# flo-audio/flo

Measured on AMD Instinct MI355X. Metric: Msamples/s encoded (44.1k stereo, q=high), higher is better.
Workload: dtype f32

## Files before the change

### diag/lds_model.py

```python
#!/usr/bin/env python3
import argparse
import re
from collections import Counter

import numpy as np

N, HOP, NB = 2048, 1024, 25
SLOT_CAP = 96
ROW = 1024
EDGES = np.array([0, 100, 200, 300, 400, 510, 630, 770, 920, 1080, 1270, 1480, 1720, 2000, 2320, 2700, 3150, 3700,
                  4400, 5300, 6400, 7700, 9500, 12000, 15500, 20500], dtype=np.float32)

R_WIN, R_TW, R_F1, R_F2, R_LANE, R_KEEP, R_DST, R_S10 = 0, 8, 12, 16, 20, 21, 25, 32


def bands(rate):
    res = np.float32(rate) / np.float32(N)
    band = []
    for k in range(HOP):
        f = (np.float32(k) + np.float32(0.5)) * res
        b = NB - 1
        for i in range(1, 26):
            if f < EDGES[i]:
                b = i - 1
                break
        band.append(b)
    return band


def band_tables(rate):
    band = bands(rate)
    lane_bnd, lane_slot0, slot_band = [0] * 64, [0] * 64, []
    for j in range(64):
        lane_slot0[j] = len(slot_band)
        for e in range(16):
            k = 16 * j + e
            if e == 15 or band[k + 1] != band[k]:
                lane_bnd[j] |= 1 << e
                slot_band.append(band[k])
    dirty = 0
    for m in lane_bnd:
        dirty |= m
    band_slot0, s = [], 0
    for b in range(NB):
        band_slot0.append(s)
        while s < len(slot_band) and slot_band[s] == b:
            s += 1
    band_slot0.append(s)
    return lane_bnd, lane_slot0, band_slot0, dirty


G128 = [[0, 1, 2, 3, 12, 13, 14, 15] + list(range(20, 28)), [4, 5, 6, 7, 8, 9, 10, 11, 16, 17, 18, 19] + list(range(28, 32))]
G128 = G128 + [[l + 32 for l in g] for g in G128]
G32 = [list(range(0, 32)), list(range(32, 64))]


def contig(n):
    return [list(range(i, i + n)) for i in range(0, 64, n)]


RULES = {
    "ds_read_b32": [(G32, 1, 32)], "ds_write_b32": [(G32, 1, 32)], "ds_write_b16": [(G32, 1, 32)],
    "ds_read_b64": [(G32, 2, 64)], "ds_read_b128": [(G128, 4, 64)],
    "ds_read2_b32": [(G32, 1, 32), (G32, 1, 32)], "ds_write2_b32": [(G32, 1, 32), (G32, 1, 32)],
    "ds_read2_b64": [(contig(16), 2, 32), (contig(16), 2, 32)],
    "ds_write_b64": [(contig(16), 2, 32)], "ds_write_b128": [(contig(8), 4, 32)],
    "ds_write2_b64": [(contig(16), 2, 32), (contig(16), 2, 32)],
}
SKIP_EMPTY = False
GATHER_MASKS = False


def cost(kind, addrs):
    acc = RULES[kind]
    lists = addrs if len(acc) == 2 else [addrs]
    cyc = base = 0
    for (groups, dw, nbank), ad in zip(acc, lists):
        for g in groups:
            per_bank = {}
            for l in g:
                if ad[l] is None:
                    continue
                for i in range(dw):
                    d = ad[l] // 4 + i
                    per_bank.setdefault(d % nbank, set()).add(d)
            if SKIP_EMPTY and not per_bank:
                continue
            cyc += max([len(v) for v in per_bank.values()] or [1])
            base += 1
    return cyc, cyc - base


def lanes(f):
    return [f(l) for l in range(64)]


def sites(rate, layout):
    lane_bnd, lane_slot0, band_slot0, dirty = band_tables(rate)
    row = lambda r, off=0: lanes(lambda l: r * ROW + 16 * l + off)
    uni = lambda a: lanes(lambda l: a)
    one = lambda a: [a] + [None] * 63
    S = []
    S += [("frame", "peek consumed / coef counters", "ds_read_b32", uni(0x8000))] * 2
    S += [("frame", "kRowS10 (uniform)", "ds_read_b128", uni(R_S10 * ROW))] * 2
    if layout == "old":
        S += [("frame", "rcount: kRowLane .z", "ds_read_b32", row(R_LANE, 8))]
    else:
        S += [("frame", "rcount: kRowS10 dword 64 + lane", "ds_read_b32", lanes(lambda l: R_S10 * ROW + 256 + 4 * l))]
    for ph, rr in (("fft pass 1", R_F1), ("fft pass 2", R_F2)):
        S += [(ph, "twiddle rows", "ds_read_b128", row(rr + k)) for k in range(3)]
        S += [(ph, "twiddle row 4 (.xy)", "ds_read_b64", row(rr + 3))]
    X = 0x10000
    for ka in range(8):
        S += [("fft exchange 1", "writes", "ds_write_b128", lanes(lambda l: X + 16 * ((8 * ka + (l & 7)) * 9 + (l >> 3))))]
    for r in range(8):
        S += [("fft exchange 1", "reads", "ds_read_b128", lanes(lambda l: X + 16 * (l * 9 + r)))]
    T = X + 16000
    S += [("masking pass", "ts_ready peek", "ds_read_b32", uni(0x8004))]
    S += [("masking pass", "ts (tl, sf)", "ds_write2_b32", [lanes(lambda l: T + 16 * (l & 31) + 4 * (l >> 5) + o if (l & 31) < 25 else None) for o in (0, 8)])]
    S += [("masking pass", "sfwh", "ds_write_b16", lanes(lambda l: T + 1024 + 2 * l if (l & 31) < 25 else None))]
    S += [("masking pass", "alive", "ds_write_b64", one(T + 1200))]
    S += [("masking pass", "ts_ready", "ds_write_b32", one(0x8004))]
    for kb in range(8):
        S += [("fft exchange 2", "writes", "ds_write_b128", lanes(lambda l: X + 16 * (((l >> 3) + 8 * kb) * 9 + (l & 7))))]
    for r in range(8):
        S += [("fft exchange 2", "reads", "ds_read_b128", lanes(lambda l: X + 16 * (l * 9 + r)))]
    pl = lambda l: 2 * l + 2 * (l >> 3)
    for r in range(8):
        if layout == "old" or r % 2 == 0:
            if layout == "old":
                S += [("post-rotation", "twiddle rows (half rows)", "ds_read_b64", row(R_TW + r // 2, 8 * (r & 1)))]
            elif layout != "carry":
                S += [("post-rotation", "twiddle rows", "ds_read_b128", row(R_TW + r // 2))]
        S += [("post-rotation", "transpose writes (2m)", "ds_write_b64", lanes(lambda l: X + 8 * (pl(l) + 144 * r)))]
        S += [("post-rotation", "transpose writes (1023-2m)", "ds_write_b64", lanes(lambda l: X + 8 * (1149 - pl(l) - 144 * r)))]
    for q in range(8):
        S += [("post-rotation", "transpose reads", "ds_read_b128", lanes(lambda l: X + 16 * (9 * l) + 16 * q))]
    S += [("band statistics", "coef_ready", "ds_write_b32", one(0x8008))]
    es = [e for e in range(16) if (dirty >> e) & 1]
    if layout == "old":
        for rr in (R_KEEP, R_DST):
            for g in range(4):
                comp = [e - 4 * g for e in es if 4 * g <= e < 4 * g + 4 and (rr == R_DST or e < 15)]
                i = 0
                while i < len(comp):
                    if i + 1 < len(comp) and comp[i + 1] == comp[i] + 1 and comp[i] % 2 == 1:
                        S += [("band statistics", "keep / dst rows (dword pieces)", "ds_read2_b32", [row(rr + g, 4 * comp[i]), row(rr + g, 4 * comp[i] + 4)])]
                        i += 2
                    elif i + 1 < len(comp) and comp[i + 1] == comp[i] + 1:
                        S += [("band statistics", "keep / dst rows (dword pieces)", "ds_read_b64", row(rr + g, 4 * comp[i]))]
                        i += 2
                    else:
                        S += [("band statistics", "keep / dst rows (dword pieces)", "ds_read_b32", row(rr + g, 4 * comp[i]))]
                        i += 1
    elif layout == "new":
        S += [("band statistics", "keep / dst rows (whole rows)", "ds_read_b128", row(rr + g)) for rr in (R_KEEP, R_DST) for g in range(4)]
    SL = X + 9216
    masks = layout in ("masks", "carry")
    for e in es:
        def dst(l, e=e, off=0):
            m = lane_bnd[l]
            if (m >> e) & 1:
                return SL + 16 * (lane_slot0[l] + bin(m & ((1 << e) - 1)).count("1")) + off
            return None if masks else SL + 16 * (SLOT_CAP + l)
        if masks and e == 15:
            S += [("band statistics", "slot store (element 15, all lanes)", "ds_write_b128", lanes(dst))]
        elif masks:
            S += [("band statistics", "slot stores (closing lanes)", "ds_write2_b64", [lanes(dst), lanes(lambda l: dst(l, off=8))])]
        else:
            S += [("band statistics", "slot stores", "ds_write_b128", lanes(dst))]
    zero = SLOT_CAP + 64
    for u in range(12):
        def src(l, u=u):
            b = min(l & 31, 24)
            bs0 = band_slot0[b] + (l >> 5)
            bs1 = band_slot0[b + 1] if (l & 31) < 25 else 0
            s = bs0 + 2 * u
            if masks and GATHER_MASKS and not bs0 + 2 * 4 * (u // 4) < bs1:
                return None
            return SL + 16 * (s if s < bs1 else zero)
        S += [("band statistics", "slot gathers", "ds_read_b128", lanes(src))]
    for r in range(8):
        S += [("fold", "window rows", "ds_read_b128", row(R_WIN + r))]
    if layout == "old":
        for k in range(4):
            S += [("fold", "twiddle rows (read2_b64)", "ds_read2_b64", [row(R_TW + k), row(R_TW + k, 8)])]
    elif layout != "carry":
        S += [("fold", "twiddle rows", "ds_read_b128", row(R_TW + k)) for k in range(4)]
    return S


def isa_mix(path):
    txt = open(path).read().split("\n")
    start = next(i for i, t in enumerate(txt) if re.match(r"^_ZN3flo20lossy_chain2q_kernelILb0ELj(\d+)ELb0EE.*:", t)
                 and "Lj65535E" not in t)
    body = txt[start:]
    e = next(i for i, t in enumerate(body) if re.match(r"^\.LBB\d+_\d+:.*_clEjS\d_S\d_S\d_S\d_\.exit", t))
    a = max(i for i, t in enumerate(body[:e]) if re.match(r"^\.LBB\d+_\d+:\s+; %\.lr\.ph\d*$", t))
    lab = body[e].split(":")[0]
    c = next(i for i, t in enumerate(body) if i > a and re.search(r"s_cbranch\w*\s+" + re.escape(lab) + r"\b", t))
    b = next(i for i, t in enumerate(body) if i > e and re.match(r"^\.LBB", t))
    mix, cold = Counter(), Counter()
    for i in range(a, b):
        m = re.search(r"\b(ds_[a-z0-9_]+)", body[i])
        if m:
            (cold if c <= i < e else mix)[m.group(1)] += 1
    return mix, cold


def main():
    ap = argparse.ArgumentParser()
    ap.add_argument("--rate", type=int, default=44100)
    ap.add_argument("--layout", default="old", choices=["old", "new", "masks", "carry"])
    ap.add_argument("--skip-empty", action="store_true")
    ap.add_argument("--gather-masks", action="store_true")
    ap.add_argument("--isa")
    a = ap.parse_args()
    global SKIP_EMPTY, GATHER_MASKS
    SKIP_EMPTY, GATHER_MASKS = a.skip_empty, a.gather_masks
    S = sites(a.rate, a.layout)
    tab = {}
    tot_c = tot_x = 0
    for ph, site, kind, ad in S:
        c, x = cost(kind, ad)
        k = (ph, site, kind)
        n, cc, xx = tab.get(k, (0, 0, 0))
        tab[k] = (n + 1, cc + c, xx + x)
        tot_c += c
        tot_x += x
    print(f"{'phase':16} {'site':38} {'instruction':14} {'n':>3} {'array':>6} {'conflict':>8}")
    for (ph, site, kind), (n, c, x) in tab.items():
        print(f"{ph:16} {site:38} {kind:14} {n:3d} {c:6d} {x:8d}")
    print(f"{'transform wave, one stereo frame':70} {len(S):3d} {tot_c:6d} {tot_x:8d}")
    if a.isa:
        mix, cold = isa_mix(a.isa)
        model = Counter(kind for _, _, kind, _ in S)
        print("ISA mix (one frame):", dict(sorted(mix.items())), " cold loop (not run at this rate):", dict(cold))
        print("model mix          :", dict(sorted(model.items())))


if __name__ == "__main__":
    main()
```

### flo_amd/csrc/lossy_device.hpp

```cpp
#pragma once
#include <hip/hip_runtime.h>
#include <stdint.h>

#include "pack_rows.h"

namespace flo {


struct LossyDevTables {
    const float4 *pack;
    const float4 *pack_g;
    const float4 *pack_ext;
    const float *ath_db;
    const uint8_t *band;
    const float *band_count;
    const float *s10d;
    const uint32_t *lane_bnd;
    const uint32_t *lane_slot0;
    const uint32_t *band_slot0;
    int max_band_slots;
    uint32_t dirty;
    float smr_thr;
    int q_transparent;
};
// ... 325 lines not shown
template <int CH>
__device__ __forceinline__ void post_rotate_transpose(const int lane, const float (&zr)[CH][8], const float (&zi)[CH][8],
                                                      float (*coef)[kCoefFloats], float (&c)[CH][16],
                                                      const LossyDevTables &T) {
#pragma unroll
    for (int r = 0; r < 8; r++) {
        const int m = lane + 64 * r;
        const float4 t4 = T.pack[(kRowTw + (r >> 1)) * 64 + lane];
        const float2 w = (r & 1) ? make_float2(t4.z, t4.w) : make_float2(t4.x, t4.y);
        const int k0 = 2 * m, k1 = 1023 - 2 * m;
        const int p0 = k0 + 4 * (k0 >> 5), p1 = k1 + 4 * (k1 >> 5);
#pragma unroll
        for (int ch = 0; ch < CH; ch++) {
            float R = fmaf(-zi[ch][r], w.y, -(zr[ch][r] * w.x));
            float I = fmaf(zi[ch][r], w.x, -(zr[ch][r] * w.y));
            coef[ch][p0] = R;
            coef[ch][p1] = I;
        }
    }
    wave_sync();
#pragma unroll
    for (int ch = 0; ch < CH; ch++) {
        const float4 *p = reinterpret_cast<const float4 *>(&coef[ch][16 * lane + 4 * (lane >> 1)]);
#pragma unroll
        for (int q = 0; q < 4; q++) {
            float4 v = p[q];
            c[ch][4 * q + 0] = v.x;
            c[ch][4 * q + 1] = v.y;
            c[ch][4 * q + 2] = v.z;
            c[ch][4 * q + 3] = v.w;
        }
    }
    wave_sync();
}

typedef float v2f __attribute__((ext_vector_type(2)));
typedef float v4f __attribute__((ext_vector_type(4)));
__device__ __forceinline__ v4f pack_row_v(const float4 *p) {
    v4f v = *reinterpret_cast<const v4f *>(p);
    asm("" : "+v"(v));
    return v;
}
__device__ __forceinline__ v2f fma2(v2f a, v2f b, v2f c) { return __builtin_elementwise_fma(a, b, c); }
__device__ __forceinline__ v2f fma2_na_hi_nc(v2f a, v2f w, v2f c) {
    v2f r;
    asm("v_pk_fma_f32 %0, %1, %2, %3 op_sel:[0,1,0] op_sel_hi:[1,1,1] neg_lo:[1,0,1] neg_hi:[1,0,1]" : "=v"(r) : "v"(a), "v"(w), "v"(c));
    return r;
}
__device__ __forceinline__ v2f fma2_a_hi_c(v2f a, v2f w, v2f c) {
    v2f r;
    asm("v_pk_fma_f32 %0, %1, %2, %3 op_sel:[0,1,0] op_sel_hi:[1,1,1]" : "=v"(r) : "v"(a), "v"(w), "v"(c));
    return r;
}
__device__ __forceinline__ v2f mul2_hi(v2f a, v2f w) {
    v2f r;
    asm("v_pk_mul_f32 %0, %1, %2 op_sel:[0,1] op_sel_hi:[1,1]" : "=v"(r) : "v"(a), "v"(w));
    return r;
}
__device__ __forceinline__ v2f fma2_a_hi_nc(v2f a, v2f w, v2f c) {
    v2f r;
    asm("v_pk_fma_f32 %0, %1, %2, %3 op_sel:[0,1,0] op_sel_hi:[1,1,1] neg_lo:[0,0,1] neg_hi:[0,0,1]" : "=v"(r) : "v"(a), "v"(w), "v"(c));
    return r;
}
__device__ __forceinline__ v2f mul2_lo(v2f a, v2f w) {
    v2f r;
    asm("v_pk_mul_f32 %0, %1, %2 op_sel:[0,0] op_sel_hi:[1,0]" : "=v"(r) : "v"(a), "v"(w));
    return r;
}
__device__ __forceinline__ v2f fma2_a_lo_nc(v2f a, v2f w, v2f c) {
    v2f r;
    asm("v_pk_fma_f32 %0, %1, %2, %3 op_sel:[0,0,0] op_sel_hi:[1,0,1] neg_lo:[0,0,1] neg_hi:[0,0,1]" : "=v"(r) : "v"(a), "v"(w), "v"(c));
    return r;
}
__device__ __forceinline__ v2f splat2(float x) { return (v2f){x, x}; }

constexpr int kXch4 = 64 * kXchStride;
constexpr int kCoef2 = 1024 + 2 * 64;

__device__ __forceinline__ void dft8_2(v2f *xr, v2f *xi) {
    const v2f s = splat2(0.70710678118654752440f);
    v2f a0r = xr[0] + xr[4], a0i = xi[0] + xi[4];
    v2f a1r = xr[0] - xr[4], a1i = xi[0] - xi[4];
    v2f a2r = xr[2] + xr[6], a2i = xi[2] + xi[6];
    v2f a3r = xr[2] - xr[6], a3i = xi[2] - xi[6];
    v2f a4r = xr[1] + xr[5], a4i = xi[1] + xi[5];
    v2f a5r = xr[1] - xr[5], a5i = xi[1] - xi[5];
    v2f a6r = xr[3] + xr[7], a6i = xi[3] + xi[7];
    v2f a7r = xr[3] - xr[7], a7i = xi[3] - xi[7];
    v2f b0r = a0r + a2r, b0i = a0i + a2i;
    v2f b2r = a0r - a2r, b2i = a0i - a2i;
    v2f b1r = a1r + a3i, b1i = a1i - a3r;
    v2f b3r = a1r - a3i, b3i = a1i + a3r;
    v2f c0r = a4r + a6r, c0i = a4i + a6i;
    v2f c2r = a4r - a6r, c2i = a4i - a6i;
    v2f c1r = a5r + a7i, c1i = a5i - a7r;
    v2f c3r = a5r - a7i, c3i = a5i + a7r;
    const v2f e1r = c1r + c1i, e1i = c1i - c1r;
    const v2f e3r = c3i - c3r, e3i = c3r + c3i;
    xr[0] = b0r + c0r; xi[0] = b0i + c0i;
    xr[4] = b0r - c0r; xi[4] = b0i - c0i;
    xr[1] = fma2(e1r, s, b1r); xi[1] = fma2(e1i, s, b1i);
    xr[5] = fma2(-e1r, s, b1r); xi[5] = fma2(-e1i, s, b1i);
    xr[2] = b2r + c2i; xi[2] = b2i - c2r;
    xr[6] = b2r - c2i; xi[6] = b2i + c2r;
    xr[3] = fma2(e3r, s, b3r); xi[3] = fma2(-e3i, s, b3i);
    xr[7] = fma2(-e3r, s, b3r); xi[7] = fma2(e3i, s, b3i);
}

__device__ __forceinline__ void cmul_2(v2f &xr, v2f &xi, float wr, float wi) {
    const v2f WR = splat2(wr), WI = splat2(wi);
    v2f r = fma2(xr, WR, -(xi * WI));
    v2f i = fma2(xr, WI, xi * WR);
    xr = r;
    xi = i;
}
__device__ __forceinline__ void cmul_2_pair(v2f &xr, v2f &xi, v2f w) {
    const v2f WR = splat2(w.x);
    v2f r = fma2(xr, WR, -mul2_hi(xi, w));
    v2f i = fma2_a_hi_c(xr, w, xi * WR);
    xr = r;
    xi = i;
}

struct NoShadow { __device__ __forceinline__ void operator()() const {} };
template <typename F = NoShadow>
__device__ __forceinline__ void fft512_2(const int lane, v2f (&zr)[8], v2f (&zi)[8], float4 *x4, const LossyDevTables &T, F &&shadow = F()) {
    dft8_2(zr, zi);
#pragma unroll
    for (int kk = 0; kk < 4; kk++) {
        const float4 w = T.pack[(kRowF1 + kk) * 64 + lane];
        cmul_2(zr[2 * kk + 1], zi[2 * kk + 1], w.x, w.y);
        if (kk < 3) cmul_2_pair(zr[2 * kk + 2], zi[2 * kk + 2], (v2f){w.z, w.w});
    }
    {
        const int nb = lane >> 3, nc = lane & 7;
#pragma unroll
        for (int ka = 0; ka < 8; ka++) x4[(8 * ka + nc) * kXchStride + nb] = make_float4(zr[ka].x, zr[ka].y, zi[ka].x, zi[ka].y);
        wave_sync();
#pragma unroll
        for (int r = 0; r < 8; r++) {
            const float4 v = x4[lane * kXchStride + r];
            zr[r] = (v2f){v.x, v.y};
            zi[r] = (v2f){v.z, v.w};
        }
        shadow();
        wave_sync();
    }
    dft8_2(zr, zi);
#pragma unroll
    for (int kk = 0; kk < 4; kk++) {
        const float4 w = T.pack[(kRowF2 + kk) * 64 + lane];
        cmul_2(zr[2 * kk + 1], zi[2 * kk + 1], w.x, w.y);
        if (kk < 3) cmul_2_pair(zr[2 * kk + 2], zi[2 * kk + 2], (v2f){w.z, w.w});
    }
    {
        const int ka = lane >> 3, nc = lane & 7;
#pragma unroll
        for (int kb = 0; kb < 8; kb++) x4[(ka + 8 * kb) * kXchStride + nc] = make_float4(zr[kb].x, zr[kb].y, zi[kb].x, zi[kb].y);
        wave_sync();
#pragma unroll
        for (int r = 0; r < 8; r++) {
            const float4 v = x4[lane * kXchStride + r];
            zr[r] = (v2f){v.x, v.y};
            zi[r] = (v2f){v.z, v.w};
        }
        wave_sync();
    }
    dft8_2(zr, zi);
}

__device__ __forceinline__ void load_half_fast_2(const int lane, const float *__restrict__ pcm, long long s0, v2f (&he)[8], v2f (&ho)[8]) {
    const char *base0 = reinterpret_cast<const char *>(pcm + s0 * 2);
    const char *base1 = base0 + 4096;
    const unsigned va = 16u * (unsigned)lane, vb = 16u * (unsigned)(63 - lane);
#pragma unroll
    for (int r = 0; r < 8; r++) {
        const int rr = r & 3;
        const char *pe = (r < 4 ? base1 : base0) + va + 1024 * rr;
        const char *po = (r < 4 ? base0 : base1) + vb + (3080 - 1024 * rr);
        const float2 a = *reinterpret_cast<const float2 *>(pe);
        const float2 b = *reinterpret_cast<const float2 *>(po);
        he[r] = (v2f){a.x, a.y};
        ho[r] = (v2f){b.x, b.y};
    }
}

__device__ __forceinline__ void fold_2(const int lane, const v2f (&ae)[8], const v2f (&ao)[8], const v2f (&be)[8], const v2f (&bo)[8],
                                       v2f (&zr)[8], v2f (&zi)[8], const LossyDevTables &T) {
    float4 t4;
#pragma unroll
    for (int r = 0; r < 8; r++) {
        const float4 ww = T.pack[(kRowWin + r) * 64 + lane];
        const v2f wae = splat2(ww.x), wao = splat2(ww.y), wbe = splat2(ww.z);
        const v2f whi = {ww.z, ww.w};
        if (!(r & 1)) t4 = pack_row(&T.pack[(kRowTw + (r >> 1)) * 64 + lane]);
        const v2f wx = splat2((r & 1) ? t4.z : t4.x);
        const v2f thi = {t4.z, t4.w};
        v2f re, im;
        if (r < 4) {
            re = fma2_na_hi_nc(bo[r], whi, be[r] * wbe);
            im = fma2(ao[r], wao, -(ae[r] * wae));
        } else {
            re = fma2(-ao[r], wao, ae[r] * wae);
            im = fma2_na_hi_nc(bo[r], whi, be[r] * wbe);
        }
        if (r & 1) {
            zr[r] = fma2_na_hi_nc(im, thi, re * wx);
            zi[r] = fma2_a_hi_nc(re, thi, im * wx);
        } else {
            const v2f wy = splat2(t4.y);
            zr[r] = fma2(-im, wy, -(re * wx));
            zi[r] = fma2(re, wy, -(im * wx));
        }
    }
}

__device__ __forceinline__ void post_rotate_transpose_2(const int lane, const v2f (&zr)[8], const v2f (&zi)[8], float2 *c2,
                                                        v2f (&c)[16], const LossyDevTables &T) {
    const int pl = 2 * lane + 2 * (lane >> 3);
    float2 *const w0 = c2 + pl;
    float2 *const w1 = c2 + (1149 - 7 * 144) - pl;
    float4 t4;
#pragma unroll
    for (int r = 0; r < 8; r++) {
        if (!(r & 1)) t4 = pack_row(&T.pack[(kRowTw + (r >> 1)) * 64 + lane]);
        const v2f wx = splat2((r & 1) ? t4.z : t4.x);
        v2f R, I;
        if (r & 1) {
            const v2f thi = {t4.z, t4.w};
            R = fma2_na_hi_nc(zi[r], thi, zr[r] * wx);
            I = fma2(zi[r], wx, -mul2_hi(zr[r], thi));
        } else {
            const v2f wy = splat2(t4.y);
            R = fma2(-zi[r], wy, -(zr[r] * wx));
            I = fma2(zi[r], wx, -(zr[r] * wy));
        }
        w0[144 * r] = make_float2(R.x, R.y);
        w1[144 * (7 - r)] = make_float2(I.x, I.y);
    }
    wave_sync();
    const float4 *p = reinterpret_cast<const float4 *>(&c2[18 * lane]);
#pragma unroll
    for (int q = 0; q < 8; q++) {
        const float4 v = p[q];
        c[2 * q] = (v2f){v.x, v.y};
        c[2 * q + 1] = (v2f){v.z, v.w};
    }
    wave_sync();
}

__device__ __forceinline__ v2f fold_a_part(const int r, const v2f he, const v2f ho, const float4 ww) {
    const v2f wae = splat2(ww.x), wao = splat2(ww.y);
    return r < 4 ? fma2(ho, wao, -(he * wae)) : fma2(-ho, wao, he * wae);
}
__device__ __forceinline__ void fold_carry_init_2(const int lane, v2f (&acar)[8], const LossyDevTables &T) {
#pragma unroll
    for (int r = 0; r < 8; r++) acar[r] = fold_a_part(r, splat2(0.f), splat2(0.f), T.pack[(kRowWin + r) * 64 + lane]);
}
__device__ __forceinline__ void fold_carry_2(const int lane, const v2f (&ne)[8], const v2f (&no)[8], v2f (&acar)[8],
                                             const v4f (&tw)[4], v2f (&zr)[8], v2f (&zi)[8], const LossyDevTables &T) {
#pragma unroll
    for (int r = 0; r < 8; r++) {
        const float4 ww = T.pack[(kRowWin + r) * 64 + lane];
        const v2f wbe = splat2(ww.z);
        const v2f whi = {ww.z, ww.w};
        const v2f t2 = (r & 1) ? tw[r >> 1].zw : tw[r >> 1].xy;
        const v2f bp = fma2_na_hi_nc(no[r], whi, ne[r] * wbe);
        const v2f re = r < 4 ? bp : acar[r], im = r < 4 ? acar[r] : bp;
        zr[r] = fma2_na_hi_nc(im, t2, mul2_lo(re, t2));
        zi[r] = fma2_a_hi_nc(re, t2, mul2_lo(im, t2));
        acar[r] = fold_a_part(r, ne[r], no[r], ww);
    }
}

__device__ __forceinline__ void post_rotate_transpose_2_tw(const int lane, const v2f (&zr)[8], const v2f (&zi)[8], float2 *c2,
                                                           v2f (&c)[16], const v4f (&tw)[4]) {
    const int pl = 2 * lane + 2 * (lane >> 3);
    float2 *const w0 = c2 + pl;
    float2 *const w1 = c2 + (1149 - 7 * 144) - pl;
#pragma unroll
    for (int r = 0; r < 8; r++) {
        const v2f t2 = (r & 1) ? tw[r >> 1].zw : tw[r >> 1].xy;
        const v2f R = fma2_na_hi_nc(zi[r], t2, mul2_lo(zr[r], t2));
        const v2f I = fma2_a_lo_nc(zi[r], t2, mul2_hi(zr[r], t2));
        w0[144 * r] = make_float2(R.x, R.y);
        w1[144 * (7 - r)] = make_float2(I.x, I.y);
    }
    wave_sync();
    const float4 *p = reinterpret_cast<const float4 *>(&c2[18 * lane]);
#pragma unroll
    for (int q = 0; q < 8; q++) {
        const float4 v = p[q];
        c[2 * q] = (v2f){v.x, v.y};
        c[2 * q + 1] = (v2f){v.z, v.w};
    }
    wave_sync();
}

struct LaneConst {
    float rcount;
};

__device__ __forceinline__ void load_lane_const(const int lane, LaneConst &L, const LossyDevTables &T) {
    L.rcount = T.pack[kRowLane * 64 + lane].z;
}

// ... 994 lines not shown
```

### flo_amd/csrc/lossy_kernels.hip

```cpp
#include <assert.h>
#include <stdlib.h>

#include <mutex>
#include <set>
#include <type_traits>
#include <utility>

#include "chain2q_roles.hpp"
#include "crc_device.hpp"
#include "lossy_device.hpp"
#include "lossy_kernels.hpp"
#include "../../include/flo_synth.h"

#ifndef FLO_SKIP
#define FLO_SKIP 0
#endif
#define FLO_KEEP(x) asm volatile("" ::"v"(x))
#ifdef FLO_STAMPS
#define STAMP(i)                                                                                  \
    do {                                                                                          \
        __builtin_amdgcn_sched_barrier(0);                                                        \
        unsigned long long t_;                                                                    \
        asm volatile("s_memtime %0\n\ts_waitcnt lgkmcnt(0)" : "=s"(t_)::"memory");              \
        __builtin_amdgcn_sched_barrier(0);                                                        \
// ... 466 lines not shown
            for (unsigned h = 0; h < hops; h++) {
                const int ln = lane_id_opaque();
                const uint32_t g = fbase + h;
                if (pturn) {
                    if ((h + pturn) & 1u) __builtin_amdgcn_s_setprio(kPackerPrio);
                    else __builtin_amdgcn_s_setprio(kPackerPrio + 1);
                }
                auto take_next = [&]() __attribute__((always_inline)) {
                    if (!have && (uint32_t)__builtin_amdgcn_readfirstlane((int)peek_counter(&cs.coef_ready)) >= g + 2) {
#pragma unroll
                        for (int k = 0; k < 8; k++) cf[k] = *reinterpret_cast<const lds_v4f *>((uintptr_t)(cf_a + 1152u * (uint32_t)k));
                        set_counter(&cs.consumed, g + 2);
                        have = true;
                    }
                };
                if (!have) {
                    wait_counter(&cs.coef_ready, g + 1);
#pragma unroll
                    for (int k = 0; k < 8; k++) cf[k] = *reinterpret_cast<const lds_v4f *>((uintptr_t)(cf_a + 1152u * (uint32_t)k));
                    set_counter(&cs.consumed, g + 1);
                }
                STAMP(0);
#ifdef FLO_STAMPS
                const unsigned long long st_frame0 = st_last;
#endif
                wait_counter(&cs.ts_ready, g + 1);
                STAMP(5);
                const uint32_t par = g & 1u;
                const uint32_t sfw_both = cs.sfwh[par][ln >> 5][ln & 31];
                const uint32_t alive = (uint32_t)__builtin_amdgcn_readfirstlane((int)(cs.alive[par][0] | cs.alive[par][1]));
                uint32_t xd[2][8];
#if (FLO_SKIP & 64) == 0
                const uint32_t visited = (uint32_t)__ballot((alive & blk_l) != 0u) & 0xFFu;
                if (par) quantise_nat<512>(cf, ts_a, athn, visited, xd);
                else quantise_nat<0>(cf, ts_a, athn, visited, xd);
#else
                const uint32_t visited = 0xFFu;
#pragma unroll
                for (int q = 0; q < 8; q++) { xd[0][q] = __float_as_uint(cf[q].x) & alive & 0x00010001u; xd[1][q] = __float_as_uint(cf[q].y) & blk_l & 0x00010001u; }
#endif
#ifdef FLO_STAMPS
                st_sum[7] += (unsigned long long)__builtin_popcount(visited);
#endif
                have = false;
                take_next();
                STAMP(1);
                if (DBG && A.dbg_q) {
#pragma unroll
                    for (int ch = 0; ch < 2; ch++) {
                        uint32_t *dq = reinterpret_cast<uint32_t *>(A.dbg_q + ((frame0 + h) * 2 + ch) * 1024);
#pragma unroll
                        for (int k = 0; k < 8; k++) dq[64 * k + ln] = xd[ch][k];
                    }
                }
                if (ln < (int)pend) stage[ln] = (uint8_t)tailb;
                uint8_t *f = stage + pend;
                const uint32_t f_a = (uint32_t)(uintptr_t)f;
                if ((ln & 31) < 25) {
                    uint8_t *p = f + 12 + 50 * (ln >> 5) + 2 * (ln & 31);
                    lds_st8<0>(p, sfw_both);
                    lds_st8<1>(p, sfw_both >> 8);
                }
                uint32_t tot[2];
                uint32_t pos = 112;
#pragma unroll
                for (int ch = 0; ch < 2; ch++) {
#if (FLO_SKIP & 32) == 0
                    uint32_t t = sparse_item_pack(ln, xd[ch], f_a + pos + 4u, tab_a, visited);
#ifdef FLO_STAMPS
                    if (t == kSparseFallback) st_sum[6] += 1;
#endif
                    if (t == kSparseFallback) t = sparse_block_pack(ln, xd[ch], f_a + pos + 4u, tab_a, visited);
#else
                    uint32_t t = 3u + ((xd[ch][0] | xd[ch][3]) & 1u);
                    FLO_KEEP(xd[ch][1]); FLO_KEEP(xd[ch][2]); FLO_KEEP(xd[ch][4]); FLO_KEEP(xd[ch][5]); FLO_KEEP(xd[ch][6]); FLO_KEEP(xd[ch][7]);
#endif
                    if (t == kSparseFallback) {
                        uint32_t *scr = reinterpret_cast<uint32_t *>(stage + 2560);
#pragma unroll
                        for (int k = 0; k < 8; k++) scr[64 * k + ln] = xd[ch][k];
                        wave_sync();
                        const uint4 x0 = reinterpret_cast<const uint4 *>(scr)[2 * ln], x1 = reinterpret_cast<const uint4 *>(scr)[2 * ln + 1];
                        wave_sync();
                        const uint32_t xs[8] = {x0.x, x0.y, x0.z, x0.w, x1.x, x1.y, x1.z, x1.w};
                        int q[1][16];
                        uint32_t hi[8];
#pragma unroll
                        for (int k = 0; k < 8; k++) {
                            hi[k] = xs[k] >> 16;
                            q[0][2 * k] = (int)xs[k];
                            q[0][2 * k + 1] = (int)hi[k];
                        }
                        SparsePlan P[1];
                        sparse_plan_m(ln, nonzero_mask16_packed(xs, hi), P[0]);
                        uint8_t *const dsts[1] = {f + pos + 4};
                        const uint32_t trash[1] = {(uint32_t)((stage + kFrameCap + 64 + 2 * ln) - dsts[0])};
                        sparse_emit_n<1>(ln, q, P, dsts, trash);
                        t = P[0].total;
                    }
                    tot[ch] = t;
                    pos += 4u + t;
                    if (ch == 0) take_next();
                    STAMP(2 + ch);
                }
                const uint32_t flen = pos, blob_len = flen - 10;
                {
                    const uint32_t i = (uint32_t)ln;
                    const uint32_t w0 = 0x000400FDu, w1 = blob_len << 16, w2 = (blob_len >> 16) | 0x02000000u;
                    uint32_t wv4 = i < 4u ? w0 : (i < 8u ? w1 : w2);
                    wv4 = i < 12u ? wv4 : (i < 16u ? tot[0] : tot[1]);
                    const uint32_t off = i < 12u ? i : (i < 16u ? 112u - 12u + i : 116u - 16u + tot[0] + i);
                    const uint32_t bv = wv4 >> (8u * (i & 3u));
                    if (i < 20u) lds_st8<0>(f + off, bv);
                    if (ln == 0) A.frame_size[frame0 + h] = flen;
                }
                wave_sync();
                take_next();
                const uint32_t haveb = pend + flen;
                const uint32_t n16 = haveb >> 4;
                const uint4 *src = reinterpret_cast<const uint4 *>(stage);
                uint4 *dst = reinterpret_cast<uint4 *>(gout + written);
                for (uint32_t i = ln; i < n16; i += 64) dst[i] = src[i];
                pend = haveb & 15u;
                tailb = (ln < (int)pend) ? stage[(n16 << 4) + ln] : 0u;
                written += (unsigned long long)n16 << 4;
                wave_sync();
                STAMP(4);
#ifdef FLO_STAMPS
                {
                    const unsigned long long busy = st_last - st_frame0;
                    if (busy > 12000) { st_sum[9] += busy; st_sum[10] += 1; }
                    if (busy > 20000) { st_sum[11] += busy; st_sum[12] += 1; }
                }
#endif
            }
            if (lane < (int)pend) gout[written + lane] = (uint8_t)tailb;
            if (lane == 0) A.clip_bytes[clip] = written + pend;
            done_clip = clip;
            done_bytes = written + pend;
            STAMPS_RECORD(1);
            fbase += hops;
        }
    }

    LossyDevTables T = A.T;
    T.pack = reinterpret_cast<const float4 *>(lds_raw);
    uint32_t so_pre[12], slot_first;
    band_stats_2_prepare(lane, cs.slot, A.T.pack, so_pre, slot_first);
    unsigned long long close[16];
    band_stats_2_masks<DIRTY>(masks, close);
    float ath_floor = masks->band_ath_floor[lane & 31];
    asm volatile("" : "+v"(ath_floor));
    v4f tw[4];
    if (!COEFFS) {
#pragma unroll
        for (int k = 0; k < 4; k++) tw[k] = pack_row_v(&T.pack[(kRowTw + k) * 64 + lane]);
    }
    for (;;) {
        wait_counter(&cs.clip_seq, ++seq);
        const unsigned clip = (unsigned)__builtin_amdgcn_readfirstlane((int)cs.clip_cur);
        if (clip >= (unsigned)A.n_clips) return;
        const unsigned hops = A.clip_hops[clip];
        const unsigned long long frame0 = A.clip_frame0[clip];
        const float *pcm = A.pcm + A.clip_off[clip];

        float prev = 0.f;
        v2f ne[8], no[8], acar[8];
        if (!COEFFS) {
            fold_carry_init_2(lane_id_opaque(), acar, T);
            load_half_fast_2(lane_id_opaque(), pcm, 0, ne, no);
        }
        STAMPS_BEGIN();
        v2f zr[8], zi[8];
        if (!COEFFS) fold_carry_2(lane_id_opaque(), ne, no, acar, tw, zr, zi, T);
        float pend_e = 0.f, pend_m = 0.f;
        auto mask_publish = [&](const int ln, const uint32_t gp, const unsigned hp, const float energy1, const float bmax1,
                                const float rcount, const float4 sd0, const float4 sd1) __attribute__((always_inline)) {
            const int bnd = ln & 31, up = ln >> 5;
#if (FLO_SKIP & 16) == 0
            const float bm = bmax1;
            const float sfv1 = bm > 1e-10f ? __fdiv_rn(30000.0f, bm) : 1.0f;
            const uint32_t sfw1 = sf_word(sfv1);
            const float a = spread_threshold_2r(ln, energy1, rcount, sd0, sd1, T);
            const float sl = max_raw(a, prev * 0.7f);
            prev = sl;
            const float tl1 = masking_amplitude(sl, T.smr_thr);
#else
            const float bm = bmax1, tl1 = energy1 * 1e-3f + rcount + sd0.x + sd1.y, sfv1 = bm * 100.f + 1.f;
            const uint32_t sfw1 = __float_as_uint(tl1) >> 16;
#endif
            const unsigned long long al = __ballot(bnd < 25 && bm > tl1 && bm > ath_floor);
            if (bnd < 25) {
                typedef __attribute__((address_space(3))) float lds_f32;
                const uint32_t ts_s = (uint32_t)__builtin_amdgcn_readfirstlane((int)(uint32_t)(uintptr_t)cs.ts[gp & 1u]);
                lds_f32 *tp = reinterpret_cast<lds_f32 *>((uintptr_t)(ts_s + 16u * (uint32_t)bnd + 4u * (uint32_t)up));
                tp[0] = tl1;
                tp[2] = sfv1;
                cs.sfwh[gp & 1u][up][bnd] = (uint16_t)sfw1;
            }
            if (ln == 0) {
                cs.alive[gp & 1u][0] = (uint32_t)al;
                cs.alive[gp & 1u][1] = (uint32_t)(al >> 32);
            }
            if (DBG && A.dbg_sfw && bnd < 25) A.dbg_sfw[((frame0 + hp) * 2 + up) * 25 + bnd] = (unsigned short)sfw1;
            set_counter(&cs.ts_ready, gp + 1);
        };
        auto frame_body = [&](const unsigned h) __attribute__((always_inline)) {
            const int ln = lane_id_opaque();
            const uint32_t g = fbase + h;
            FLO_MARK("frame_begin");
            const uint32_t consumed_early = peek_counter(&cs.consumed);
            const float4 sd0 = T.pack[kRowS10 * 64], sd1 = T.pack[kRowS10 * 64 + 1];
            const float rcount = reinterpret_cast<const float *>(T.pack + kRowS10 * 64)[64 + ln];
            v2f c[16];
            if (COEFFS) {
#pragma unroll
                for (int q = 0; q < 4; q++) {
                    const float4 v0 = reinterpret_cast<const float4 *>(A.in_coeffs + ((frame0 + h) * 2 + 0) * 1024 + 16 * ln)[q];
                    const float4 v1 = reinterpret_cast<const float4 *>(A.in_coeffs + ((frame0 + h) * 2 + 1) * 1024 + 16 * ln)[q];
                    c[4 * q] = (v2f){v0.x, v1.x}; c[4 * q + 1] = (v2f){v0.y, v1.y};
                    c[4 * q + 2] = (v2f){v0.z, v1.z}; c[4 * q + 3] = (v2f){v0.w, v1.w};
                }
                if ((uint32_t)__builtin_amdgcn_readfirstlane((int)consumed_early) < g) wait_counter(&cs.consumed, g);
                float4 *p = reinterpret_cast<float4 *>(&cs.u.coef2[18 * ln]);
#pragma unroll
                for (int q = 0; q < 8; q++) p[q] = make_float4(c[2 * q].x, c[2 * q].y, c[2 * q + 1].x, c[2 * q + 1].y);
                wave_sync();
            } else {
                load_half_fast_2(ln, pcm, (long long)(h + 1) * 1024, ne, no);
                FLO_MARK("prefetch_done");
                STAMP(1);
                if ((uint32_t)__builtin_amdgcn_readfirstlane((int)consumed_early) < g) wait_counter(&cs.consumed, g);
                STAMP(7);
#if (FLO_SKIP & 8) == 0
                fft512_2(ln, zr, zi, cs.u.xch4, T, [&]() __attribute__((always_inline)) {
                    if (h > 0) mask_publish(ln, g - 1u, h - 1u, pend_e, pend_m, rcount, sd0, sd1);
                });
#else
                if (h > 0) mask_publish(ln, g - 1u, h - 1u, pend_e, pend_m, rcount, sd0, sd1);
#endif
                FLO_MARK("fft_done");
                STAMP(2);
#if (FLO_SKIP & 4) == 0
                post_rotate_transpose_2_tw(ln, zr, zi, cs.u.coef2, c, tw);
#else
#pragma unroll
                for (int e = 0; e < 8; e++) { c[2 * e] = zr[e]; c[2 * e + 1] = zi[e]; }
#endif
                FLO_MARK("postrot_done");
                STAMP(3);
                if (DBG && A.dbg_coeffs) {
#pragma unroll
                    for (int ch = 0; ch < 2; ch++) {
                        float *d = A.dbg_coeffs + ((frame0 + h) * 2 + ch) * 1024 + 16 * ln;
#pragma unroll
                        for (int e = 0; e < 16; e++) d[e] = ch ? c[e].y : c[e].x;
                    }
                }
            }
            set_counter(&cs.coef_ready, g + 1);
            float energy1, bmax1;
#if (FLO_SKIP & 1) == 0
            band_stats_2<DIRTY, true, true>(ln, c, cs.slot, T, energy1, bmax1, so_pre, close, slot_first);
#else
            energy1 = c[0].x + c[5].y;
            bmax1 = c[1].x + c[7].y;
#endif
            FLO_MARK("bandstats_done");
            STAMP(4);
            if (COEFFS) {
                mask_publish(ln, g, h, energy1, bmax1, rcount, sd0, sd1);
            } else {
                pend_e = energy1, pend_m = bmax1;
#if (FLO_SKIP & 128) == 0
                fold_carry_2(ln, ne, no, acar, tw, zr, zi, T);
#else
#pragma unroll
                for (int r = 0; r < 8; r++) { zr[r] = acar[r] + ne[r]; zi[r] = acar[r] - no[r]; }
#endif
            }
            FLO_MARK("frame_end");
            STAMP(5);
        };
        for (unsigned h = 0; h < hops; h++) frame_body(h);
        if (!COEFFS && hops) {
            const int ln = lane_id_opaque();
            const float4 sd0 = T.pack[kRowS10 * 64], sd1 = T.pack[kRowS10 * 64 + 1];
            mask_publish(ln, fbase + hops - 1u, hops - 1u, pend_e, pend_m, reinterpret_cast<const float *>(T.pack + kRowS10 * 64)[64 + ln], sd0, sd1);
        }
        STAMPS_RECORD(0);
        fbase += hops;
    }
}

template <int CH, int STEP, bool EXACT>
__global__ __launch_bounds__(64) void lossy_frame_kernel(LossyArgs A) {
    constexpr int PASS = STEP & ~kStreamStep;
    constexpr bool STREAM = (STEP & kStreamStep) != 0;
    __shared__ WaveLds<CH> lds;
    __shared__ __attribute__((aligned(16))) uint8_t stage[kFrameCap + 64 + 256];
    const int lane = lane_id();
    const unsigned long long gframe = blockIdx.x;
    if (gframe >= A.total_frames) return;
    int lo = 0, hi = A.n_clips - 1;
    while (lo < hi) {
        int mid = (lo + hi + 1) >> 1;
        if (A.clip_frame0[mid] <= gframe) lo = mid; else hi = mid - 1;
    }
    const unsigned clip = (unsigned)lo;
    const unsigned h = (unsigned)(gframe - A.clip_frame0[clip]);
    const float *pcm = A.pcm + A.clip_off[clip];
    const long long n_sf = (long long)A.clip_nsf[clip];

    LaneConst L;
    load_lane_const(lane, L, A.T);
    if (lane < CH) lds.slots[lane][kZeroSlot] = make_float2(0.f, 0.f);
    float c[CH][16];
    if (A.in_coeffs) {
        load_coeffs<CH>(lane, c, A, gframe, 0);
    } else {
        float ae[CH][8], ao[CH][8], be[CH][8], bo[CH][8];
        load_half<CH>(lane, pcm, n_sf, A.nch, 0, (long long)(h + STREAM) * 1024 - 1024, ae, ao);
        load_half<CH>(lane, pcm, n_sf, A.nch, 0, (long long)(h + STREAM) * 1024, be, bo);
        mdct_frame<CH>(lane, ae, ao, be, bo, lds, A.T, c);
    }
    FrameState<CH> st;
    int q[CH][16];
    uint32_t sfw[CH];
    SparsePlan P[CH];
    if (PASS == 1) {
#pragma unroll
        for (int ch = 0; ch < CH; ch++) st.prev[ch] = 0.f;
        analyse_frame<CH, true, EXACT>(lane, c, lds, L, A, A.T, 0, st, gframe, q, sfw, P);
        if (lane < 25) {
#pragma unroll
            for (int ch = 0; ch < CH; ch++) mark_inf_level(A, clip, (unsigned)ch, (unsigned)lane, h, A.a_t[(gframe * A.nch + ch) * 32 + lane]);
        }
        return;
    }
    store_coeffs_dbg<CH>(lane, c, A, gframe, 0);
#pragma unroll
    for (int ch = 0; ch < CH; ch++) st.prev[ch] = lane < 25 ? A.s_prev[(gframe * A.nch + ch) * 32 + lane] : 0.f;
    analyse_frame<CH, false, EXACT>(lane, c, lds, L, A, A.T, 0, st, gframe, q, sfw, P);
    uint32_t tot[2];
    tot[0] = P[0].total;
    tot[1] = P[CH - 1].total;
    const uint32_t flen = emit_frame<CH>(lane, stage, CH, 0, tot, sfw, P, q);
    wave_sync();
    if (lane == 0) A.frame_size[gframe] = flen;
    const uint32_t n16 = (flen + 15) >> 4;
    const uint4 *src = reinterpret_cast<const uint4 *>(stage);
    uint4 *dst = reinterpret_cast<uint4 *>(A.slots + gframe * (unsigned long long)A.slot_bytes);
    for (uint32_t i = lane; i < n16; i += 64) dst[i] = src[i];
}

constexpr int kScanBlock = 64;
struct QuantOnlyLds {
    float4 ts[32];
    uint32_t qh[2][512];
};
template <int STEP, bool FROMCOEF = false>
__global__ __launch_bounds__(64) void lossy_frame2x_kernel(LossyArgs A) {
    constexpr int PASS = STEP & ~kStreamStep;
    constexpr bool STREAM = (STEP & kStreamStep) != 0;
    constexpr bool kSmall = PASS == 2 && FROMCOEF;
    __shared__ typename std::conditional<kSmall, QuantOnlyLds, StereoLds>::type lds;
    __shared__ __attribute__((aligned(16))) uint8_t stage[PASS == 2 ? kFrameCap + 64 + 256 : 16];
    static_assert(sizeof(StereoLds) >= 2 * 512 * 4, "the integers of both channels fit the analysis buffers");
    uint32_t (*qh)[512];
    float4 *ts_tab;
    if constexpr (kSmall) {
        qh = lds.qh;
        ts_tab = lds.ts;
    } else {
        qh = reinterpret_cast<uint32_t (*)[512]>(&lds);
        ts_tab = lds.u.a.ts;
    }
    __shared__ uint32_t runtab[PASS == 2 ? kRunTabEntries : 1];
    const int lane = lane_id();
    const unsigned long long gframe = blockIdx.x;
    if (gframe >= A.total_frames) return;
    int lo = 0, hi = A.n_clips - 1;
    while (lo < hi) {
        int mid = (lo + hi + 1) >> 1;
        if (A.clip_frame0[mid] <= gframe) lo = mid; else hi = mid - 1;
    }
    const unsigned clip = (unsigned)lo;
    const unsigned h = (unsigned)(gframe - A.clip_frame0[clip]);
    const float *pcm = A.pcm + A.clip_off[clip];
    const LossyDevTables &T = A.T;

    v2f c[16];
    if constexpr (kSmall) {
        const float4 *src = A.coef_t + gframe * 512ull + (unsigned)lane;
#pragma unroll
// ... 874 lines not shown
```

### profiles/phase_table.py

```python
#!/usr/bin/env python3
import collections
import re
import sys


def classify(op):
    if op.startswith("v_"):
        return "valu"
    if op.startswith("ds_"):
        return "lds"
    if op.startswith("s_waitcnt"):
        return "wait"
    if op.startswith(("global_", "buffer_", "flat_", "scratch_")):
        return "vmem"
    if op.startswith("s_load") or op.startswith("s_buffer_load"):
        return "smem"
    if op.startswith("s_"):
        return "salu"
    return None


def main():
    path = sys.argv[1]
    want = sys.argv[2] if len(sys.argv) > 2 else "lossy_chain2q_kernelILb0ELj48574ELb0EE"
    lines = open(path).read().split("\n")
    start = next(i for i, l in enumerate(lines) if l.startswith("_Z") and want in l and ":" in l.split(";")[0])
    end = next(i for i in range(start, len(lines)) if ".size" in lines[i] and want in lines[i])
    phases = collections.OrderedDict()
    cur = "pre (clip set-up, packer wave)"
    order = []
    bodies = max(1, sum(1 for l in lines[start:end] if l.strip().startswith("; MARK frame_begin")))
    last_end = max((i for i in range(start, end) if lines[i].strip().startswith("; MARK frame_end")), default=end)
    for i, l in enumerate(lines[start:end], start):
        if i == last_end + 1:
            cur = "post (behind the last frame_end)"
        s = l.strip()
        m = re.match(r"; MARK (\w+)", s)
        if m:
            cur = m.group(1)
            continue
        if not s or s.startswith((";", ".", "//")) or s.endswith(":"):
            continue
        op = s.split()[0]
        k = classify(op)
        if k is None:
            continue
        phases.setdefault(cur, collections.Counter())[k] += 1
        if cur not in order:
            order.append(cur)
    names = {"frame_begin": "prefetch (16 loads), masking rows", "prefetch_done": "fft512 x2 + masking pass (prev. frame)",
             "fft_done": "post-rotation + transpose", "postrot_done": "band_stats_2",
             "bandstats_done": "fold of the next frame (a)", "frame_end": "fold of the next frame (b), loop"}
    print(f"{'phase':32s} {'VALU':>6s} {'SALU':>6s} {'LDS':>5s} {'VMEM':>5s} {'wait':>5s}   (per stereo frame, {bodies} frame bod{'y' if bodies == 1 else 'ies'})")
    tot = collections.Counter()
    for ph in order:
        c = phases[ph]
        nm = names.get(ph, ph)
        once = ph.startswith(("pre (", "post ("))
        div = 1 if once else bodies
        row = {k: c[k] / div for k in ("valu", "salu", "lds", "vmem", "wait")}
        if not once:
            for k, v in row.items():
                tot[k] += v
        print(f"{nm:32s} {row['valu']:6.0f} {row['salu']:6.0f} {row['lds']:5.0f} {row['vmem']:5.0f} {row['wait']:5.0f}")
    print(f"{'transform wave, per frame':32s} {tot['valu']:6.0f} {tot['salu']:6.0f} {tot['lds']:5.0f} {tot['vmem']:5.0f} {tot['wait']:5.0f}")


if __name__ == "__main__":
    main()
```

Before: 719,300.

## Hold FFT twiddle rows in registers and move next-frame prefetch after FFT

```diff
diff --git a/diag/lds_model.py b/diag/lds_model.py
--- a/diag/lds_model.py
+++ b/diag/lds_model.py
@@ -108,6 +108,8 @@
     else:
         S += [("frame", "rcount: kRowS10 dword 64 + lane", "ds_read_b32", lanes(lambda l: R_S10 * ROW + 256 + 4 * l))]
     for ph, rr in (("fft pass 1", R_F1), ("fft pass 2", R_F2)):
+        if layout == "fftrows":
+            continue
         S += [(ph, "twiddle rows", "ds_read_b128", row(rr + k)) for k in range(3)]
         S += [(ph, "twiddle row 4 (.xy)", "ds_read_b64", row(rr + 3))]
     X = 0x10000
@@ -130,7 +132,7 @@
         if layout == "old" or r % 2 == 0:
             if layout == "old":
                 S += [("post-rotation", "twiddle rows (half rows)", "ds_read_b64", row(R_TW + r // 2, 8 * (r & 1)))]
-            elif layout != "carry":
+            elif layout not in ("carry", "fftrows"):
                 S += [("post-rotation", "twiddle rows", "ds_read_b128", row(R_TW + r // 2))]
         S += [("post-rotation", "transpose writes (2m)", "ds_write_b64", lanes(lambda l: X + 8 * (pl(l) + 144 * r)))]
         S += [("post-rotation", "transpose writes (1023-2m)", "ds_write_b64", lanes(lambda l: X + 8 * (1149 - pl(l) - 144 * r)))]
@@ -156,7 +158,7 @@
     elif layout == "new":
         S += [("band statistics", "keep / dst rows (whole rows)", "ds_read_b128", row(rr + g)) for rr in (R_KEEP, R_DST) for g in range(4)]
     SL = X + 9216
-    masks = layout in ("masks", "carry")
+    masks = layout in ("masks", "carry", "fftrows")
     for e in es:
         def dst(l, e=e, off=0):
             m = lane_bnd[l]
@@ -185,7 +187,7 @@
     if layout == "old":
         for k in range(4):
             S += [("fold", "twiddle rows (read2_b64)", "ds_read2_b64", [row(R_TW + k), row(R_TW + k, 8)])]
-    elif layout != "carry":
+    elif layout not in ("carry", "fftrows"):
         S += [("fold", "twiddle rows", "ds_read_b128", row(R_TW + k)) for k in range(4)]
     return S
 
@@ -211,7 +213,7 @@
 def main():
     ap = argparse.ArgumentParser()
     ap.add_argument("--rate", type=int, default=44100)
-    ap.add_argument("--layout", default="old", choices=["old", "new", "masks", "carry"])
+    ap.add_argument("--layout", default="old", choices=["old", "new", "masks", "carry", "fftrows"])
     ap.add_argument("--skip-empty", action="store_true")
     ap.add_argument("--gather-masks", action="store_true")
     ap.add_argument("--isa")
diff --git a/flo_amd/csrc/lossy_device.hpp b/flo_amd/csrc/lossy_device.hpp
--- a/flo_amd/csrc/lossy_device.hpp
+++ b/flo_amd/csrc/lossy_device.hpp
@@ -501,6 +501,57 @@
         const float4 w = T.pack[(kRowF2 + kk) * 64 + lane];
         cmul_2(zr[2 * kk + 1], zi[2 * kk + 1], w.x, w.y);
         if (kk < 3) cmul_2_pair(zr[2 * kk + 2], zi[2 * kk + 2], (v2f){w.z, w.w});
+    }
+    {
+        const int ka = lane >> 3, nc = lane & 7;
+#pragma unroll
+        for (int kb = 0; kb < 8; kb++) x4[(ka + 8 * kb) * kXchStride + nc] = make_float4(zr[kb].x, zr[kb].y, zi[kb].x, zi[kb].y);
+        wave_sync();
+#pragma unroll
+        for (int r = 0; r < 8; r++) {
+            const float4 v = x4[lane * kXchStride + r];
+            zr[r] = (v2f){v.x, v.y};
+            zi[r] = (v2f){v.z, v.w};
+        }
+        wave_sync();
+    }
+    dft8_2(zr, zi);
+}
+
+__device__ __forceinline__ void cmul_2_tw(v2f &xr, v2f &xi, v2f w) {
+    const v2f r = fma2_a_lo_nc(xr, w, mul2_hi(xi, w));
+    const v2f i = fma2_a_hi_c(xr, w, mul2_lo(xi, w));
+    xr = r;
+    xi = i;
+}
+template <typename F = NoShadow>
+__device__ __forceinline__ void fft512_2_tw(const int lane, v2f (&zr)[8], v2f (&zi)[8], float4 *x4, const v4f (&f1)[4],
+                                            const v4f (&f2)[4], F &&shadow = F()) {
+    dft8_2(zr, zi);
+#pragma unroll
+    for (int kk = 0; kk < 4; kk++) {
+        cmul_2_tw(zr[2 * kk + 1], zi[2 * kk + 1], f1[kk].xy);
+        if (kk < 3) cmul_2_tw(zr[2 * kk + 2], zi[2 * kk + 2], f1[kk].zw);
+    }
+    {
+        const int nb = lane >> 3, nc = lane & 7;
+#pragma unroll
+        for (int ka = 0; ka < 8; ka++) x4[(8 * ka + nc) * kXchStride + nb] = make_float4(zr[ka].x, zr[ka].y, zi[ka].x, zi[ka].y);
+        wave_sync();
+#pragma unroll
+        for (int r = 0; r < 8; r++) {
+            const float4 v = x4[lane * kXchStride + r];
+            zr[r] = (v2f){v.x, v.y};
+            zi[r] = (v2f){v.z, v.w};
+        }
+        shadow();
+        wave_sync();
+    }
+    dft8_2(zr, zi);
+#pragma unroll
+    for (int kk = 0; kk < 4; kk++) {
+        cmul_2_tw(zr[2 * kk + 1], zi[2 * kk + 1], f2[kk].xy);
+        if (kk < 3) cmul_2_tw(zr[2 * kk + 2], zi[2 * kk + 2], f2[kk].zw);
     }
     {
         const int ka = lane >> 3, nc = lane & 7;
diff --git a/flo_amd/csrc/lossy_kernels.hip b/flo_amd/csrc/lossy_kernels.hip
--- a/flo_amd/csrc/lossy_kernels.hip
+++ b/flo_amd/csrc/lossy_kernels.hip
@@ -642,9 +642,14 @@
     float ath_floor = masks->band_ath_floor[lane & 31];
     asm volatile("" : "+v"(ath_floor));
     v4f tw[4];
+    v4f f1[4], f2[4];
     if (!COEFFS) {
 #pragma unroll
         for (int k = 0; k < 4; k++) tw[k] = pack_row_v(&T.pack[(kRowTw + k) * 64 + lane]);
+#pragma unroll
+        for (int k = 0; k < 4; k++) f1[k] = pack_row_v(&T.pack[(kRowF1 + k) * 64 + lane]);
+#pragma unroll
+        for (int k = 0; k < 4; k++) f2[k] = pack_row_v(&T.pack[(kRowF2 + k) * 64 + lane]);
     }
     for (;;) {
         wait_counter(&cs.clip_seq, ++seq);
@@ -717,13 +722,11 @@
                 for (int q = 0; q < 8; q++) p[q] = make_float4(c[2 * q].x, c[2 * q].y, c[2 * q + 1].x, c[2 * q + 1].y);
                 wave_sync();
             } else {
-                load_half_fast_2(ln, pcm, (long long)(h + 1) * 1024, ne, no);
-                FLO_MARK("prefetch_done");
                 STAMP(1);
                 if ((uint32_t)__builtin_amdgcn_readfirstlane((int)consumed_early) < g) wait_counter(&cs.consumed, g);
                 STAMP(7);
 #if (FLO_SKIP & 8) == 0
-                fft512_2(ln, zr, zi, cs.u.xch4, T, [&]() __attribute__((always_inline)) {
+                fft512_2_tw(ln, zr, zi, cs.u.xch4, f1, f2, [&]() __attribute__((always_inline)) {
                     if (h > 0) mask_publish(ln, g - 1u, h - 1u, pend_e, pend_m, rcount, sd0, sd1);
                 });
 #else
@@ -731,6 +734,8 @@
 #endif
                 FLO_MARK("fft_done");
                 STAMP(2);
+                load_half_fast_2(ln, pcm, (long long)(h + 1) * 1024, ne, no);
+                FLO_MARK("prefetch_done");
 #if (FLO_SKIP & 4) == 0
                 post_rotate_transpose_2_tw(ln, zr, zi, cs.u.coef2, c, tw);
 #else
diff --git a/profiles/phase_table.py b/profiles/phase_table.py
--- a/profiles/phase_table.py
+++ b/profiles/phase_table.py
@@ -31,8 +31,24 @@
     order = []
     bodies = max(1, sum(1 for l in lines[start:end] if l.strip().startswith("; MARK frame_begin")))
     last_end = max((i for i in range(start, end) if lines[i].strip().startswith("; MARK frame_end")), default=end)
+    marks = [(i, re.match(r"; MARK (\w+)", lines[i].strip()).group(1)) for i in range(start, end) if lines[i].strip().startswith("; MARK ")]
+    first = {n: min(i for i, m in marks if m == n) for n in {m for _, m in marks}}
+    rotated = "frame_end" in first and "frame_begin" in first and first["frame_end"] < first["frame_begin"]
+    loop_start = post_start = None
+    if rotated:
+        label_at = lambda i: max(j for j in range(start, i + 1) if re.match(r"\.LBB\d+_\d+:", lines[j]))
+        loop_start, header = label_at(marks[0][0]), label_at(first["frame_begin"])
+        leave = next(lines[j] for j in range(header - 1, loop_start, -1) if lines[j].strip().startswith("s_cbranch"))
+        exit_label = leave.split()[1]
+        post_start = next(j for j in range(start, end) if lines[j].startswith(exit_label + ":"))
+        assert post_start > marks[-1][0], "the loop's exit lies behind its last marker"
     for i, l in enumerate(lines[start:end], start):
-        if i == last_end + 1:
+        if rotated:
+            if i == loop_start:
+                cur = marks[-1][1]
+            elif i == post_start:
+                cur = "post (behind the frame loop)"
+        elif i == last_end + 1:
             cur = "post (behind the last frame_end)"
         s = l.strip()
         m = re.match(r"; MARK (\w+)", s)
@@ -48,8 +64,13 @@
         phases.setdefault(cur, collections.Counter())[k] += 1
         if cur not in order:
             order.append(cur)
-    names = {"frame_begin": "prefetch (16 loads), masking rows", "prefetch_done": "fft512 x2 + masking pass (prev. frame)",
-             "fft_done": "post-rotation + transpose", "postrot_done": "band_stats_2",
+    if rotated:
+        seq = [m for _, m in marks]
+        k = seq.index("frame_begin")
+        prog = seq[k:] + seq[:k]
+        order = [o for o in order if o.startswith("pre (")] + [m for m in prog if m in order] + [o for o in order if o.startswith("post (")]
+    names = {"frame_begin": "masking rows, fft512 x2 + masking pass (prev. frame)", "fft_done": "prefetch (16 loads)",
+             "prefetch_done": "post-rotation + transpose", "postrot_done": "band_stats_2",
              "bandstats_done": "fold of the next frame (a)", "frame_end": "fold of the next frame (b), loop"}
     print(f"{'phase':32s} {'VALU':>6s} {'SALU':>6s} {'LDS':>5s} {'VMEM':>5s} {'wait':>5s}   (per stereo frame, {bodies} frame bod{'y' if bodies == 1 else 'ies'})")
     tot = collections.Counter()
```

New measurement: 744,700 (median of 6 runs). +3.5%, better.
